# Xjh-UCAS/TAM-TR

Hardware: AMD Instinct MI355X
Metric: images/sec fwd+bwd @640x640 bs=16/GPU (higher is better)
Workload: dtype bf16

## Files before the change

### include/tamtr_hip.h

```cpp
#ifndef TAMTR_HIP_H
#define TAMTR_HIP_H

#include <stdint.h>

#ifdef __cplusplus
extern "C" {
#endif

#define TAMTR_F32 0
#define TAMTR_BF16 1

#define TAMTR_OK 0
#define TAMTR_EINVAL (-1)
#define TAMTR_EUNSUP (-2)
#define TAMTR_ELAUNCH (-3)

int tamtr_abi_version(void);

int tamtr_maxsigmoid_gate_fwd(const void* x, const float* gk, const float* bias, const void* v, void* out, float* aw,
                              int32_t* arg, int B, int nh, int hc, int HW, int T, float scale, int dtype, void* stream);

int tamtr_maxsigmoid_gate_bwd(const void* dout, const void* x, const float* gk, const void* v, const float* aw,
                              const int32_t* arg, void* dx, void* dv, float* dlogit, int B, int nh, int hc, int HW, int T,
                              float scale, int dtype, void* stream);
// ... 13 lines not shown
int tamtr_msdeform_attn_fwd(const void* value, const int32_t* shapes_host, const float* loc, const float* aw, void* out,
                            int B, int L, int M, int D, int Q, int nl, int P, int dtype, void* stream);

int tamtr_msdeform_attn_bwd(const void* gout, const void* value, const int32_t* shapes_host, const float* loc,
                            const float* aw, float* gvalue, float* gloc, float* gaw, int B, int L, int M, int D, int Q,
                            int nl, int P, int dtype, void* stream);

int tamtr_msdeform_attn_bwd_sorted(const void* gout, const void* value, const int32_t* shapes_host, const float* loc,
                                   const float* aw, void* gvalue, float* gloc, float* gaw, float* colw, int B, int L, int M,
                                   int D, int Q, int nl, int P, long long ldg, int dtype, void* stream);

int tamtr_contrastive_logits_fwd(const void* x, const float* w, const float* logit_scale, const float* bias, float* logits,
                                 float* xinv, float* winv, int B, int Q, int K, int C, int dtype, void* stream);

int tamtr_contrastive_bwd_slabs(int Q);
int tamtr_contrastive_logits_bwd(const float* g, const void* x, const float* w, const float* logit_scale, const float* xinv,
                                 const float* winv, void* dx, float* dwhat, int B, int Q, int K, int C, int dtype,
                                 void* stream);

int tamtr_linear_bf16(const void* X, const void* W, const float* bias, void* Y, int M, int N, int K, void* stream);

int tamtr_selfattn_fwd(const void* q, const void* k, const void* v, const uint32_t* mask_bits, void* o, float* lse, int B,
                       int Q, int nh, int dh, int ldq, int ldk, int ldv, int dtype, void* stream);
int tamtr_selfattn_bwd(const void* go, const void* q, const void* k, const void* v, const void* o, const float* lse,
                       const uint32_t* mask_bits, void* gq, void* gk, void* gv, float* delta_ws, int B, int Q, int nh, int dh,
                       int ldq, int ldk, int ldv, int dtype, void* stream);

int tamtr_selective_scan_chunk(void);
int tamtr_selective_scan_fwd(const float* u, const float* delta, const float* A, const float* Bm, const float* Cm,
                             const float* D, const float* dbias, float* y, float* hstate, int B, int K, int Dk, int N, int L,
                             int xmode, void* stream);
int tamtr_selective_scan_bwd_slabs(int Dk);
int tamtr_selective_scan_row_sums(void);
int tamtr_selective_scan_bwd(const float* gy, const float* u, const float* delta, const float* A, const float* Bm,
                             const float* Cm, const float* D, const float* dbias, const float* hstate, float* gu,
                             float* gdelta, float* grow, float* gB, float* gC, float* ws, int B, int K, int Dk, int N, int L,
                             int xmode, void* stream);

int tamtr_selective_scan_dtproj_fwd(const void* u, const float* dtr, const float* Wdt, const float* A, const float* Bm,
                                    const float* Cm, const float* D, const float* dbias, void* y, float* hstate, int B, int K,
                                    int Dk, int N, int R, int L, int xmode, int planes_bf16, void* stream);
int tamtr_selective_scan_dtproj_bwd(const void* gy, const void* u, const float* dtr, const float* Wdt, const float* A,
                                    const float* Bm, const float* Cm, const float* D, const float* dbias, const float* hstate,
                                    void* gu, void* gdelta_ws, float* gdtr, float* grow, float* gB, float* gC, float* ws, int B,
                                    int K, int Dk, int N, int R, int L, int xmode, int bf16_flags, void* stream);

int tamtr_lsap_assign(const float* cost, const int32_t* group_sizes_host, int bs, int nq, int G, int64_t* batch_idx,
                      int64_t* query_idx, int64_t* gt_idx, void* stream);

int tamtr_cpam_fwd(const void* x, const void* p, void* out, float* s2, int32_t* arg, int B, int C, int H, int W, int dtype,
                   void* stream);

int tamtr_cpam_bwd(const void* gout, const void* x, const void* p, const float* s2, const int32_t* arg, void* dx_direct,
                   void* du_ws, void* dp, int B, int C, int H, int W, int dtype, void* stream);

int tamtr_cpam_cl_fwd(const void* x, void* p, uint8_t* code, void* out, float* s2, int32_t* arg, int B, int C, int H, int W, int dtype, void* stream);
int tamtr_cpam_cl_bwd(const void* gout, const void* x, const void* p, const uint8_t* code, const float* s2, const int32_t* arg, void* dxd_ws,
                      void* du_ws, void* dp_ws, void* dx, int B, int C, int H, int W, int dtype, void* stream);

int tamtr_dwconv_silu_cross_fwd(const void* x, long long x_pixel_stride, const float* weight, const float* bias, void* u2, int B,
                                int D, int H, int W, int dtype, int plane_dtype, void* stream);
int tamtr_dwconv_tiles(int H, int W);
int tamtr_dwconv_silu_cross_bwd(const void* g2, const void* x, long long x_pixel_stride, const float* weight, const float* bias,
                                void* gx, long long gx_pixel_stride, float* ws, int B, int D, int H, int W, int dtype, int plane_dtype,
                                void* stream);

int tamtr_cross_merge_fwd(const void* y4, float* ymT, int B, int D, int H, int W, int plane_dtype, void* stream);
int tamtr_cross_merge_bwd(const float* gymT, void* g2, int B, int D, int H, int W, int plane_dtype, void* stream);

int tamtr_ln_gate_blocks(long long ntok);
int tamtr_ln_gate_fwd(const float* x, const void* xz, long long xz_token_stride, const float* gamma, const float* beta, void* out,
                      float* stats, long long ntok, int D, float eps, int dtype, void* stream);
int tamtr_ln_gate_bwd(const void* gout, const float* x, const void* xz, long long xz_token_stride, const float* gamma,
                      const float* beta, const float* stats, float* gx, void* gxz, float* partials, long long ntok, int D, int dtype,
                      void* stream);

int tamtr_sum_n(const void* const* src, int n, void* out, long long n_elems, int dtype, void* stream);

int tamtr_colsum_blocks(long long M);
int tamtr_colsum_bf16(const void* X, float* partial, long long M, int N, void* stream);
int tamtr_slab_sum_rows(const void* in, float* out, int R, long long C, int dtype, void* stream);
int tamtr_dw_slices(long long M, int N, int K);
int tamtr_dw_bf16(const void* dY, const void* X, float* part, int with_db, long long M, int N, int K, void* stream);
int tamtr_fold_add(const float* g4, const void* m0, const void* m1, float* out, int B, long long n, int dtype, void* stream);

int tamtr_layernorm_fwd(const void* x, const float* gamma, const float* beta, void* out, float* stats, long long ntok, int D,
                        float eps, int dtype, void* stream);
int tamtr_layernorm_bwd(const void* gout, const void* x, const float* gamma, const float* stats, void* gx, float* partials,
                        long long ntok, int D, int dtype, void* stream);

int tamtr_bn_slices(int B, int HW);
int tamtr_bn_act_fwd(const void* x, const float* gamma, const float* beta, float* running_mean, float* running_var, void* y,
                     float* mean_rstd, float* partials, int B, int C, int HW, float eps, float momentum, int act, int dtype, void* stream);
int tamtr_bn_act_bwd(const void* gy, const void* x, const float* gamma, const float* beta, const float* mean_rstd, void* gx,
                     float* ggamma, float* gbeta, float* partials, int B, int C, int HW, int act, int dtype, void* stream);

int tamtr_bncl_blocks(long long N, int C, int dtype);
int tamtr_bncl_act_fwd(const void* x, const float* gamma, const float* beta, float* running_mean, float* running_var, const void* residual,
                       void* y, float* mean_rstd, float* partials, long long N, int C, float eps, float momentum, int act, int dtype,
                       void* stream);
int tamtr_bncl_stats(const void* x, float* running_mean, float* running_var, float* mean_rstd, float* partials, long long N, int C, float eps,
                     float momentum, int dtype, void* stream);
int tamtr_bncl2_act_fwd(const void* x1, const float* gamma1, const float* beta1, float* running_mean1, float* running_var1, const void* x2,
                        const float* gamma2, const float* beta2, float* running_mean2, float* running_var2, void* y, float* mean_rstd,
                        float* partials, long long N, int C, float eps, float momentum, int act, int dtype, void* stream);
int tamtr_bncl2_act_bwd(const void* gy, long long ldgy, const void* x1, const void* x2, const float* gamma1, const float* beta1,
                        const float* gamma2, const float* beta2, const float* mean_rstd, void* gx1, void* gx2, float* ggamma1, float* gbeta1,
                        float* ggamma2, float* gbeta2, float* partials, long long N, int C, int act, int dtype, void* stream);
int tamtr_bncl_act_bwd(const void* gy, long long ldgy, const void* x, const float* gamma, const float* beta, const float* mean_rstd,
                       void* gx, float* ggamma, float* gbeta, float* partials, long long N, int C, int act, int dtype, void* stream);

int tamtr_relayout(const void* src, void* dst, int B, int C, int HW, int ld, int to_nhwc, int dtype, void* stream);
int tamtr_resample2(const void* src, void* dst, int B, int H, int W, int C, int mode, int dtype, void* stream);
int tamtr_copy_rows(const void* src, long long lds, void* dst, long long ldd, long long N, int C, int dtype, void* stream);
int tamtr_cat_rows(const void* const* src, const long long* lds, const int* C, int n, void* dst, long long ldd, long long N, int dtype,
                   void* stream);

int tamtr_maxpool_out(int n, int k, int s, int p);
int tamtr_maxpool_fwd(const void* x, void* y, uint8_t* code, int B, int C, int H, int W, int k, int s, int p, int nhwc, int dtype,
                      void* stream);
int tamtr_maxpool_bwd(const void* gy, const uint8_t* code, const void* addend, void* gx, int B, int C, int H, int W, int k, int s, int p, int nhwc, int dtype,
                      void* stream);

int tamtr_img_augment_u8(const uint8_t* src, const double* inv_affine, const uint8_t* luts, const int32_t* flags, float* out, int B,
                         int SH, int SW, int H, int W, int border, void* stream);

int tamtr_optim_chunk(void);
int tamtr_optim_step(const void* const* p, const void* const* m, const void* const* v, const void* const* e, const void* const* shadow, float* step,
                     const long long* numel,
                     const unsigned char* group, const int* chunk_tensor, const long long* chunk_off, const void* const* grads, int ntensors,
                     int nchunks, float* partial, float* normcoef, const float* lr, const float* wd, int ngroups, float beta1, float beta2, float eps,
                     float max_norm, float ema_decay, int do_ema, void* stream);

int tamtr_xproj_dw_slices(int L);
int tamtr_xproj_fwd(const void* u2, const void* wcat, float* dtr, float* Bs, float* Cs, int B, int D, int L, int R, int plane_dtype, void* stream);
int tamtr_xproj_bwd_dx(const void* gu, const float* gdtr, const float* gB, const float* gC, const void* wT, void* gu2, int B, int D, int L, int R,
                       int plane_dtype, void* stream);
int tamtr_xproj_bwd_dw(const void* u2, const float* gdtr, const float* gB, const float* gC, float* part, int B, int D, int L, int R, int plane_dtype,
                       void* stream);

int tamtr_detr_blocks(int rows_per_layer);
int tamtr_detr_layers_fwd(const float* pb, const float* ps, const float* gt_bboxes, const long long* gt_cls, const long long* li, const long long* bi,
                          const long long* si, const long long* gi, int Lr, int B, int nq, int nc, int n, long long* tgt, float* score, float* pair_l1,
                          float* pair_riou, float* partial, float g_class, float g_bbox, float g_giou, float* out, void* stream);
int tamtr_detr_layers_bwd(const float* pb, const float* ps, const float* gt_bboxes, const long long* li, const long long* bi, const long long* si,
                          const long long* gi, const long long* tgt, const float* score, const float* up, int Lr, int B, int nq, int nc, int n,
                          float g_class, float g_bbox, float g_giou, float* gpb, float* gps, void* stream);
int tamtr_detr_match_cost(const float* ps, const float* pb, const float* gt_bboxes, const long long* gt_cls, long long rows, int nc, int G, float g_class,
                          float g_bbox, float g_giou, float alpha, float gamma, float* C, void* stream);

int tamtr_bncl_act_seg_fwd(const void* x, const float* gamma, const float* beta, float* running_mean, float* running_var, void* y, long long seg_rows,
                           long long seg_pitch, float* mean_rstd, float* partials, long long N, int C, float eps, float momentum, int act, int dtype,
                           void* stream);
int tamtr_bncl_act_seg_bwd(const void* gy, long long seg_rows, long long seg_pitch, const void* x, const float* gamma, const float* beta,
                           const float* mean_rstd, void* gx, float* ggamma, float* gbeta, float* partials, long long N, int C, int act, int dtype,
                           void* stream);

int tamtr_box_refine_fwd(const float* delta, const float* ref, float* out, long long n, void* stream);
int tamtr_box_refine_bwd(const float* gout, const float* out, const float* ref, float* gdelta, float* gref, long long n, void* stream);

int tamtr_graph_capture_census(void* stream, int* counts, int n_types);

int tamtr_detect_postprocess(const void* preds, int dtype, int B, int nq, int nd, const int32_t* orig_hw, float conf, float iou,
                             int single_cls, float max_wh, const int32_t* classes, int n_classes, float* out, int32_t* keep,
                             int32_t* counts, void* stream);

// ... 80 lines not shown
```

### tam-tr_amd/_lib.py

```python
import ctypes
import os
from ctypes import c_float, c_int, c_longlong, c_void_p

_HERE = os.path.dirname(os.path.abspath(__file__))
LIB_PATH = os.environ.get('TAMTR_HIP_LIB') or os.path.join(_HERE, 'csrc', 'libtamtr_hip.so')
ABI_VERSION = 36

F32, BF16 = 0, 1
_ERR = {-1: 'TAMTR_EINVAL (bad argument)', -2: 'TAMTR_EUNSUP (shape/dtype outside what the kernels are built for)',
        -3: 'TAMTR_ELAUNCH (HIP launch error)'}


class TamtrHipError(RuntimeError):
    pass


_P, _I, _F, _LL, _D = c_void_p, c_int, c_float, c_longlong, ctypes.c_double
_SIGS = {
    'tamtr_abi_version': [],
    'tamtr_maxsigmoid_gate_fwd': [_P, _P, _P, _P, _P, _P, _P, _I, _I, _I, _I, _I, _F, _I, _P],
    'tamtr_maxsigmoid_gate_bwd': [_P, _P, _P, _P, _P, _P, _P, _P, _P, _I, _I, _I, _I, _I, _F, _I, _P],
    'tamtr_msdeform_attn_fwd': [_P, _P, _P, _P, _P, _I, _I, _I, _I, _I, _I, _I, _I, _P],
    'tamtr_msdeform_attn_bwd': [_P, _P, _P, _P, _P, _P, _P, _P, _I, _I, _I, _I, _I, _I, _I, _I, _P],
    'tamtr_msdeform_attn_bwd_sorted': [_P, _P, _P, _P, _P, _P, _P, _P, _P, _I, _I, _I, _I, _I, _I, _I, _LL, _I, _P],
    'tamtr_contrastive_logits_fwd': [_P, _P, _P, _P, _P, _P, _P, _I, _I, _I, _I, _I, _P],
    'tamtr_contrastive_logits_bwd': [_P, _P, _P, _P, _P, _P, _P, _P, _I, _I, _I, _I, _I, _P],
    'tamtr_contrastive_bwd_slabs': [_I],
    'tamtr_linear_bf16': [_P, _P, _P, _P, _I, _I, _I, _P],
    'tamtr_selfattn_fwd': [_P, _P, _P, _P, _P, _P, _I, _I, _I, _I, _I, _I, _I, _I, _P],
    'tamtr_selfattn_bwd': [_P] * 11 + [_I, _I, _I, _I, _I, _I, _I, _I, _P],
    'tamtr_selective_scan_chunk': [],
    'tamtr_selective_scan_fwd': [_P, _P, _P, _P, _P, _P, _P, _P, _P, _I, _I, _I, _I, _I, _I, _P],
    'tamtr_selective_scan_bwd_slabs': [_I],
    'tamtr_selective_scan_row_sums': [],
    'tamtr_selective_scan_bwd': [_P] * 15 + [_I, _I, _I, _I, _I, _I, _P],
    'tamtr_selective_scan_dtproj_fwd': [_P] * 10 + [_I] * 8 + [_P],
    'tamtr_selective_scan_dtproj_bwd': [_P] * 17 + [_I] * 8 + [_P],
    'tamtr_lsap_assign': [_P, _P, _I, _I, _I, _P, _P, _P, _P],
    'tamtr_img_augment_u8': [_P, _P, _P, _P, _P, _I, _I, _I, _I, _I, _I, _P],
    'tamtr_cpam_fwd': [_P, _P, _P, _P, _P, _I, _I, _I, _I, _I, _P],
    'tamtr_cpam_cl_fwd': [_P, _P, _P, _P, _P, _P, _I, _I, _I, _I, _I, _P],
    'tamtr_cpam_bwd': [_P] * 8 + [_I, _I, _I, _I, _I, _P],
    'tamtr_cpam_cl_bwd': [_P] * 10 + [_I, _I, _I, _I, _I, _P],
    'tamtr_dwconv_silu_cross_fwd': [_P, _LL, _P, _P, _P, _I, _I, _I, _I, _I, _I, _P],
    'tamtr_dwconv_tiles': [_I, _I],
    'tamtr_cross_merge_fwd': [_P, _P, _I, _I, _I, _I, _I, _P],
    'tamtr_cross_merge_bwd': [_P, _P, _I, _I, _I, _I, _I, _P],
    'tamtr_ln_gate_blocks': [_LL],
    'tamtr_bn_slices': [_I, _I],
    'tamtr_maxpool_out': [_I, _I, _I, _I],
    'tamtr_maxpool_fwd': [_P, _P, _P, _I, _I, _I, _I, _I, _I, _I, _I, _I, _P],
    'tamtr_maxpool_bwd': [_P, _P, _P, _P, _I, _I, _I, _I, _I, _I, _I, _I, _I, _P],
    'tamtr_sum_n': [_P, _I, _P, _LL, _I, _P],
    'tamtr_colsum_blocks': [_LL],
    'tamtr_colsum_bf16': [_P, _P, _LL, _I, _P],
    'tamtr_fold_add': [_P, _P, _P, _P, _I, _LL, _I, _P],
    'tamtr_slab_sum_rows': [_P, _P, _I, _LL, _I, _P],
    'tamtr_dw_slices': [_LL, _I, _I],
    'tamtr_dw_bf16': [_P, _P, _P, _I, _LL, _I, _I, _P],
    'tamtr_graph_capture_census': [_P, _P, _I],
    'tamtr_box_refine_fwd': [_P, _P, _P, _LL, _P],
    'tamtr_box_refine_bwd': [_P, _P, _P, _P, _P, _LL, _P],
    'tamtr_bncl_act_seg_fwd': [_P, _P, _P, _P, _P, _P, _LL, _LL, _P, _P, _LL, _I, _F, _F, _I, _I, _P],
    'tamtr_bncl_act_seg_bwd': [_P, _LL, _LL, _P, _P, _P, _P, _P, _P, _P, _P, _LL, _I, _I, _I, _P],
    'tamtr_detr_blocks': [_I],
    'tamtr_detr_layers_fwd': [_P] * 8 + [_I] * 5 + [_P] * 5 + [_F, _F, _F, _P, _P],
    'tamtr_detr_layers_bwd': [_P] * 10 + [_I] * 5 + [_F, _F, _F, _P, _P, _P],
    'tamtr_detr_match_cost': [_P, _P, _P, _P, _LL, _I, _I, _F, _F, _F, _F, _F, _P, _P],
    'tamtr_xproj_dw_slices': [_I],
    'tamtr_xproj_fwd': [_P, _P, _P, _P, _P, _I, _I, _I, _I, _I, _P],
    'tamtr_xproj_bwd_dx': [_P, _P, _P, _P, _P, _P, _I, _I, _I, _I, _I, _P],
    'tamtr_xproj_bwd_dw': [_P, _P, _P, _P, _P, _I, _I, _I, _I, _I, _P],
    'tamtr_optim_chunk': [],
    'tamtr_optim_step': [_P] * 11 + [_I, _I, _P, _P, _P, _P, _I, _F, _F, _F, _F, _F, _I, _P],
    'tamtr_resample2': [_P, _P, _I, _I, _I, _I, _I, _I, _P],
    'tamtr_cat_rows': [_P, _P, _P, _I, _P, _LL, _LL, _I, _P],
    'tamtr_copy_rows': [_P, _LL, _P, _LL, _LL, _I, _I, _P],
    'tamtr_relayout': [_P, _P, _I, _I, _I, _I, _I, _I, _P],
    'tamtr_bncl_blocks': [_LL, _I, _I],
    'tamtr_bncl_act_fwd': [_P, _P, _P, _P, _P, _P, _P, _P, _P, _LL, _I, _F, _F, _I, _I, _P],
    'tamtr_bncl_stats': [_P, _P, _P, _P, _P, _LL, _I, _F, _F, _I, _P],
    'tamtr_bn_finalize': [_P, _P, _P, _P, _I, _I, _F, _F, _P],
    'tamtr_conv3x3_tiles': [_I, _I, _I],
    'tamtr_conv3x3_pack_weight': [_P, _P, _I, _I, _I, _P],
    'tamtr_conv3x3_cl_stats_fwd': [_P, _LL, _P, _P, _P, _P, _P, _P, _I, _I, _I, _I, _I, _F, _F, _P],
    'tamtr_maxsigmoid_gate_cl_fwd': [_P, _LL, _P, _P, _P, _P, _P, _P, _P, _P, _P, _P, _P, _P, _I, _I, _I, _I, _I, _F, _I, _P],
    'tamtr_bncl2_act_fwd': [_P, _P, _P, _P, _P, _P, _P, _P, _P, _P, _P, _P, _P, _LL, _I, _F, _F, _I, _I, _P],
    'tamtr_bncl2_act_bwd': [_P, _LL, _P, _P, _P, _P, _P, _P, _P, _P, _P, _P, _P, _P, _P, _P, _LL, _I, _I, _I, _P],
    'tamtr_bncl_act_bwd': [_P, _LL, _P, _P, _P, _P, _P, _P, _P, _P, _LL, _I, _I, _I, _P],
    'tamtr_bn_act_fwd': [_P, _P, _P, _P, _P, _P, _P, _P, _I, _I, _I, _F, _F, _I, _I, _P],
    'tamtr_bn_act_bwd': [_P, _P, _P, _P, _P, _P, _P, _P, _P, _I, _I, _I, _I, _I, _P],
    'tamtr_layernorm_fwd': [_P, _P, _P, _P, _P, _LL, _I, _F, _I, _P],
    'tamtr_layernorm_bwd': [_P, _P, _P, _P, _P, _P, _LL, _I, _I, _P],
    'tamtr_ln_gate_fwd': [_P, _P, _LL, _P, _P, _P, _P, _LL, _I, _F, _I, _P],
    'tamtr_ln_gate_bwd': [_P, _P, _P, _LL, _P, _P, _P, _P, _P, _P, _LL, _I, _I, _P],
    'tamtr_dwconv_silu_cross_bwd': [_P, _P, _LL, _P, _P, _P, _LL, _P, _I, _I, _I, _I, _I, _I, _P],
    'tamtr_detect_postprocess': [_P, _I, _I, _I, _I, _P, _F, _F, _I, _F, _P, _I, _P, _P, _P, _P],
    'tamtr_val_postprocess_match': [_P, _I, _I, _I, _I, _F, _F, _F, _I, _F, _P, _P, _P, _I, _P, _P, _P, _P, _P],
    'tamtr_val_confusion': [_P, _P, _I, _I, _I, _P, _P, _P, _I, _P, _F, _F, _P, _P],
    'tamtr_val_ap_tile': [],
    'tamtr_val_ap_curves': [_P, _P, _P, _I, _I, _P, _I] + [_P] * 10 + [_P],
    'tamtr_text_embed': [_P, _P, _P, _P, _LL, _I, _I, _I, _P],
    'tamtr_linear_f32': [_P, _P, _P, _P, _P, _I, _I, _I, _I, _P],
    'tamtr_text_pool_project': [_P, _P, _P, _P, _P, _P, _I, _I, _I, _I, _F, _I, _P],
    'tamtr_bytetrack_update': [_P, _P, _I, _I, _P, _P, _P, _P, _P, _I, _F, _F, _F, _D, _I, _P, _P, _P, _I, _P],
    'tamtr_bytetrack_workspace_bytes': [_I, _I],
    'tamtr_botsort_update': [_P, _P, _P, _I, _I, _P, _P, _P, _P, _P, _I, _F, _F, _F, _D, _I, _P, _P, _P, _I, _P],
    'tamtr_botsort_reid_update': [_P, _P, _P, _P, _I, _I, _P, _P, _P, _P, _P, _P, _I, _I, _F, _F, _F, _D, _I, _F, _D, _P, _P, _P, _I, _P],
    'tamtr_botsort_reid_workspace_bytes': [_I, _I],
    'tamtr_reid_rows': [_P, _I, _P, _P, _I, _I, _I, _I, _P, _P],
    'tamtr_gmc_workspace_bytes': [_I, _I, _I],
    'tamtr_gmc_workspace_offset': [_I, _I, _I, _I],
    'tamtr_gmc_state_bytes': [_I, _I],
    'tamtr_gmc_estimate': [_P, _P, _P, _I, _I, _I, _P, _P, _P, _P, _P, _P, _I, _I, _P],
    'tamtr_val_coco_match': [_P, _P, _I, _I, _I, _P, _P, _P, _I, _P, _P, _I, _P, _P, _P, _P, _I, _P],
    'tamtr_val_coco_workspace_bytes': [_I, _I, _I],
    'tamtr_val_coco_accumulate': [_P, _P, _P, _I, _I, _P, _P, _I, _P, _P, _P, _P, _P],
    'tamtr_mot_update': [_P, _P, _P, _P, _I, _I, _I, _I, _D, _P, _P, _P, _P, _P, _I, _I, _P, _I, _P],
    'tamtr_mot_end_sequence': [_I, _P, _P, _P, _P, _I, _I, _I, _P, _I, _P],
    'tamtr_mot_workspace_bytes': [_I, _I, _I, _I, _I],
    'tamtr_hota_update': [_P, _P, _P, _P, _I, _I, _I, _I, _D, _D, _P, _P, _P, _I, _P],
    'tamtr_hota_end_sequence': [_P, _D, _I, _I, _I, _I, _P, _P, _P, _I, _P],
    'tamtr_hota_workspace_bytes': [_I, _I, _I],
    'tamtr_trackmap_update': [_P, _P, _P, _P, _I, _I, _I, _I, _D, _P, _P, _P, _I, _P],
    'tamtr_trackmap_end_sequence': [_P, _I, _D, _I, _P, _P, _P, _I, _P],
    'tamtr_trackmap_workspace_bytes': [_I, _I, _I, _I, _I, _I],
}
EXPORTS = tuple(_SIGS)
_lib = None


def lib():
    global _lib
    if _lib is None:
        if not os.path.exists(LIB_PATH):
            raise TamtrHipError(f'{LIB_PATH} not found: build it with `python -c "import __graft_entry__ as g; g.build()"` '
                                '(hipcc --offload-arch=gfx950). There is no CPU fallback.')
        h = ctypes.CDLL(LIB_PATH)
        for name, args in _SIGS.items():
            fn = getattr(h, name)
            fn.argtypes = args
            fn.restype = c_int
# ... 35 lines not shown
```

### tam-tr_amd/ops.py

```python
import ctypes
import math

import torch

from . import _lib
from ._lib import call, dtype_code, ptr, require_gpu, stream_ptr
import os as _os

_PROJ_CONV_LIB = _os.environ.get('TAMTR_PROJ_CONV') == 'miopen'

_I, _F = ctypes.c_int, ctypes.c_float


def _c(t):
    return t if t.is_contiguous() else t.contiguous()


def _is_cl(t):
    return t.dim() == 4 and not t.is_contiguous() and t.is_contiguous(memory_format=torch.channels_last)


def is_cl(t):
    return _is_cl(t)

# ... 397 lines not shown
        gb = (gout.view(B * Q, M, D).float() * colw.view(B * Q, M, 1)).sum(0).view(N).to(b_dt) if ctx.needs_input_grad[2] else None
        return gx, gw, gb, None, gloc.to(loc_dt), gaw.to(aw_dt), None


def value_proj_msda_ok(x, lin, n_heads, Q, P):
    K, N = lin.in_features, lin.out_features
    return (x.is_cuda and x.dtype == torch.bfloat16 and x.dim() == 3 and lin.bias is not None and N % n_heads == 0 and K % 128 == 0 and N % 128 == 0
            and msda_sorted_ok(Q, P, N // n_heads) and not _MSDA_ATOMICS and _os.environ.get('TAMTR_VALUE_BIAS') != 'colsum')


def value_proj_msda(x, lin, n_heads, shapes, loc, aw):
    return _ValueProjMSDA.apply(x, lin.weight, lin.bias, [tuple(int(v) for v in s) for s in shapes], loc, aw, int(n_heads))


class _ContrastiveLogits(torch.autograd.Function):
    @staticmethod
    def forward(ctx, x, w, logit_scale, bias):
        require_gpu(x, w, logit_scale, bias)
        B, Q, C = x.shape
        K = w.shape[1]
        x = _c(x)
        w32 = _c(w.float())
        ls, bi = _c(logit_scale.float().reshape(1)), _c(bias.float().reshape(1))
        logits = torch.empty(B, Q, K, device=x.device, dtype=torch.float32)
        xinv = torch.empty(B, Q, device=x.device, dtype=torch.float32)
        winv = torch.empty(B, K, device=x.device, dtype=torch.float32)
        call('tamtr_contrastive_logits_fwd', ptr(x), ptr(w32), ptr(ls), ptr(bi), ptr(logits), ptr(xinv), ptr(winv), B, Q, K, C,
             dtype_code(x), stream_ptr())
        ctx.save_for_backward(x, w32, ls, bi, logits, xinv, winv)
        ctx.cfg = (w.dtype, logit_scale.dtype, logit_scale.shape, bias.dtype, bias.shape)
        return logits

    @staticmethod
    def backward(ctx, g):
        x, w32, ls, bi, logits, xinv, winv = ctx.saved_tensors
        w_dt, ls_dt, ls_shape, b_dt, b_shape = ctx.cfg
        B, Q, C = x.shape
        K = w32.shape[1]
        g = _c(g.float())
        dx = torch.empty_like(x)
        if K > 16:
            _atomic_fallback(f'the contrastive head backward sums d(what) with LDS atomics for K = {K} > 16 prompts (csrc/contrastive.hip)')
        slabs = _lib.lib().tamtr_contrastive_bwd_slabs(Q)
        dwhat = torch.empty(B, slabs, K, C, device=x.device, dtype=torch.float32)
        call('tamtr_contrastive_logits_bwd', ptr(g), ptr(x), ptr(w32), ptr(ls), ptr(xinv), ptr(winv), ptr(dx), ptr(dwhat), B, Q, K,
             C, dtype_code(x), stream_ptr())
        dwhat = dwhat.sum(1) if slabs > 1 else dwhat[:, 0]
        what = w32 * winv.unsqueeze(-1)
        dw = winv.unsqueeze(-1) * (dwhat - (dwhat * what).sum(-1, keepdim=True) * what)
        dls = (g * (logits - bi)).sum().reshape(ls_shape).to(ls_dt)
        dbias = g.sum().reshape(b_shape).to(b_dt)
        return dx, dw.to(w_dt), dls, dbias


def contrastive_logits(x, w, logit_scale, bias):
    return _ContrastiveLogits.apply(x, w, logit_scale, bias)


_SPLIT_MAX = int(_os.environ.get('TAMTR_SPLITK_MAX', '64'))


def _split_count(M, min_rows=2048, max_split=None):
    max_split = _SPLIT_MAX if max_split is None else max_split
    S = 1
    while S < max_split and M % (2 * S) == 0 and M // (2 * S) >= min_rows:
        S *= 2
    return S


_BMM_F32_OUT = None

_DW_OWN = _os.environ.get('TAMTR_DW_OWN') != '0'
_DW_OWN_MAX_ROWS = 8192


def _dw_own_slices(g2, x2):
    if not (_DW_OWN and g2.is_cuda and x2.is_cuda and g2.dtype == torch.bfloat16 and x2.dtype == torch.bfloat16 and g2.dim() == 2 and x2.dim() == 2
            and g2.shape[0] == x2.shape[0] and 0 < g2.shape[0] < _DW_OWN_MAX_ROWS and g2.is_contiguous() and x2.is_contiguous()
            and g2.data_ptr() % 16 == 0 and x2.data_ptr() % 16 == 0):
        return 0
    return _lib.lib().tamtr_dw_slices(g2.shape[0], g2.shape[1], x2.shape[1])


def _dw_own(g2, x2, S, with_db):
    M, N = g2.shape
    K = x2.shape[1]
    part = torch.empty(S, N * K + N, device=g2.device, dtype=torch.float32)
    call('tamtr_dw_bf16', ptr(g2), ptr(x2), ptr(part), int(with_db), M, N, K, stream_ptr())
    tot = slab_sum(part)
    return tot[:N * K].view(N, K), tot[N * K:]


def dw_splitk(g2, x2, min_rows=2048):
    M, N = g2.shape
    K = x2.shape[1]
    S = _dw_own_slices(g2, x2)
    if S:
        return _dw_own(g2, x2, S, False)[0]
    S = _split_count(M, min_rows)
    if S == 1:
        return (g2.t() @ x2).float()
    a, b = g2.view(S, M // S, N).transpose(1, 2), x2.view(S, M // S, K)
    global _BMM_F32_OUT
    if _BMM_F32_OUT is not False and N % 8 == 0 and K % 8 == 0:
        try:
            out = torch.bmm(a, b, out_dtype=torch.float32)
            _BMM_F32_OUT = True
            return slab_sum(out)
        except (NotImplementedError, RuntimeError, TypeError):
            if _BMM_F32_OUT:
                raise
            _BMM_F32_OUT = False
    return slab_sum(torch.bmm(a, b))


def slab_sum(t):
    R = t.shape[0]
    C = t.numel() // max(R, 1)
    if not (t.is_cuda and t.dtype in (torch.float32, torch.bfloat16) and t.is_contiguous() and R > 0 and C % 4 == 0 and t.data_ptr() % 16 == 0):
        return t.float().sum(0)
    if R == 1:
        return t[0].float()
    out = torch.empty(t.shape[1:], device=t.device, dtype=torch.float32)
    call('tamtr_slab_sum_rows', ptr(t), ptr(out), R, C, dtype_code(t), stream_ptr())
    return out


def colsum(g2):
    M, N = g2.shape
    if g2.is_cuda and g2.dtype == torch.bfloat16 and M >= 4096 and N % 8 == 0 and N <= 2048 and 256 % (N // 8) == 0 and g2.is_contiguous():
        nblk = _lib.lib().tamtr_colsum_blocks(M)
        part = torch.empty(nblk, N, device=g2.device, dtype=torch.float32)
        call('tamtr_colsum_bf16', ptr(g2), ptr(part), M, N, stream_ptr())
        return slab_sum(part)
    if g2.is_cuda and g2.dtype in (torch.float32, torch.bfloat16) and N % 4 == 0:
        return slab_sum(_c(g2))
    return g2.sum(0, dtype=torch.float32)


def bf16_shadow(p):
    s = getattr(p, '_tamtr_bf16', None)
    if s is not None:
        base = getattr(p, '_tamtr_alias_of', p)
        if s._tamtr_version == base._version and s.device == p.device and s.shape == p.shape:
            return s
    return None


def bf16_of(p):
    if p.dtype == torch.bfloat16:
        return p
    s = bf16_shadow(p)
    return s if s is not None else p.to(torch.bfloat16)


KERNEL_EVENTS = {}


def _a16(t):
    return t if t is None or t.data_ptr() % 16 == 0 else t.clone()


def _linear_bf16_fwd(x2, w16, b32):
    M, K = x2.shape
    N = w16.shape[0]
    y = torch.empty(M, N, device=x2.device, dtype=torch.bfloat16)
    x2, w16, b32 = _a16(x2), _a16(w16), _a16(b32)
    rec = KERNEL_EVENTS.get('tamtr_linear_bf16')
    if rec is not None:
        e0, e1 = torch.cuda.Event(enable_timing=True), torch.cuda.Event(enable_timing=True)
        e0.record()
    call('tamtr_linear_bf16', ptr(x2), ptr(w16), ptr(b32), ptr(y), M, N, K, stream_ptr())
    if rec is not None:
        e1.record()
        rec.append((e0, e1, 2.0 * M * N * K))
    return y


def _linear_bf16_dx(g2, w16):
    N, K = w16.shape
    if K % 128 == 0 and N % 64 == 0:
        gx = torch.empty(g2.shape[0], K, device=g2.device, dtype=torch.bfloat16)
        g2, wt = _a16(g2), _a16(_c(w16.t()))
        call('tamtr_linear_bf16', ptr(g2), ptr(wt), None, ptr(gx), g2.shape[0], K, N, stream_ptr())
        return gx
    return g2 @ w16


def _bias_rows(y, idx, b32):
    if idx.numel():
        y[:, idx] = b32.to(torch.bfloat16)


def _param_grads(g2, x2, w_dt, b_dt, need_w, need_b, min_rows=2048):
    S = _dw_own_slices(g2, x2) if need_w else 0
    if S:
        with_db = b_dt is not None and need_b
        gw, gb = _dw_own(g2, x2, S, with_db)
        return gw.to(w_dt), (gb.to(b_dt) if with_db else None)
    gw = dw_splitk(g2, x2, min_rows).to(w_dt) if need_w else None
    gb = colsum(g2).to(b_dt) if (b_dt is not None and need_b) else None
    return gw, gb


def _linear_lib_bwd(needs, gy, x, w16, x_dt, w_dt, b_dt, min_rows=2048):
    N, K = w16.shape
    g2 = _c(gy.reshape(-1, N).to(x.dtype))
    x2 = _c(x.reshape(-1, K))
    gx = (g2 @ w16).view(x.shape).to(x_dt) if needs[0] else None
    return (gx,) + _param_grads(g2, x2, w_dt, b_dt, needs[1], needs[2], min_rows)


_LM_MIN_ROWS = 256


class _LinearMaster(torch.autograd.Function):

    @staticmethod
    def forward(ctx, x, weight, bias, w16=None, b16=None):
        w16 = bf16_of(weight) if w16 is None else w16
        b16 = None if bias is None else (bf16_of(bias) if b16 is None else b16)
        x16 = x if x.dtype == torch.bfloat16 else x.to(torch.bfloat16)
        ctx.save_for_backward(x16, w16)
        ctx.cfg = (x.dtype, weight.dtype, None if bias is None else bias.dtype)
        return torch.nn.functional.linear(x16, w16, b16)

    @staticmethod
    def backward(ctx, gy):
        x16, w16 = ctx.saved_tensors
        x_dt, w_dt, b_dt = ctx.cfg
        return _linear_lib_bwd(ctx.needs_input_grad, gy, x16, w16, x_dt, w_dt, b_dt, _LM_MIN_ROWS) + (None, None)


class _LinearSplitK(torch.autograd.Function):

    @staticmethod
    def forward(ctx, x, weight, bias):
        bf = x.dtype == torch.bfloat16
        w16 = bf16_of(weight) if bf else weight.to(x.dtype)
        ctx.save_for_backward(x, w16)
        ctx.cfg = (weight.dtype, None if bias is None else bias.dtype)
        return torch.nn.functional.linear(x, w16, None if bias is None else (bf16_of(bias) if bf else bias.to(x.dtype)))

    @staticmethod
    def backward(ctx, gy):
        x, w16 = ctx.saved_tensors
        w_dt, b_dt = ctx.cfg
        return _linear_lib_bwd(ctx.needs_input_grad, gy, x, w16, x.dtype, w_dt, b_dt)


class _LinearBF16(torch.autograd.Function):

    @staticmethod
    def forward(ctx, x, weight, bias, idx):
        require_gpu(x, weight, bias)
        K = x.shape[-1]
        N = weight.shape[0]
        x2 = _c(x.reshape(-1, K))
        if x2.dtype != torch.bfloat16:
            raise _lib.TamtrHipError('linear_bf16 needs bf16 activations')
        w16 = _c(bf16_of(weight))
        b32 = _c(bias.float()) if bias is not None else None
        y = _linear_bf16_fwd(x2, w16, b32).view(*x.shape[:-1], N)
        if idx is not None:
            _bias_rows(y, idx, b32)
        ctx.save_for_backward(x2, w16, idx)
        ctx.cfg = (x.shape, weight.dtype, None if bias is None else bias.dtype)
        return y

    @staticmethod
    def backward(ctx, gy):
        x2, w16, idx = ctx.saved_tensors
        xshape, w_dt, b_dt = ctx.cfg
        N, K = w16.shape
        g2 = _c(gy.reshape(-1, N).to(torch.bfloat16))
        gx = _linear_bf16_dx(g2, w16).view(xshape) if ctx.needs_input_grad[0] else None
        masked = idx is not None and idx.numel() > 0
        gw, gb = _param_grads(g2, x2, torch.float32 if masked else w_dt, b_dt, *ctx.needs_input_grad[1:3])
        if masked and gx is not None:
            gx.index_fill_(1, idx, 0)
        if masked and gw is not None:
# ... 1941 lines not shown
```

Baseline: 218.0.

## Add split-M MFMA weight-gradient kernel for tall bf16 linear layers

Adds a new HIP kernel that computes weight gradients (dY^T X) for tall matrices (M at least 16384 rows) with bf16 inputs. It splits the rows across slices, streams tiles into LDS through a multi-stage global_load_lds ring, reads them with transposed LDS reads, accumulates with MFMA, and can fuse the bias column-sum. The per-slice fp32 partials are then reduced with the existing slab_sum. A shape heuristic routes eligible GEMMs away from the hipBLAS bmm split-K path; in exchange it adds fp32 partial buffers and heuristic tuning risk.

```diff
diff --git a/include/tamtr_hip.h b/include/tamtr_hip.h
--- a/include/tamtr_hip.h
+++ b/include/tamtr_hip.h
@@ -119,6 +119,8 @@
 int tamtr_slab_sum_rows(const void* in, float* out, int R, long long C, int dtype, void* stream);
 int tamtr_dw_slices(long long M, int N, int K);
 int tamtr_dw_bf16(const void* dY, const void* X, float* part, int with_db, long long M, int N, int K, void* stream);
+int tamtr_dw_tall_slices(long long M, int N, int K);
+int tamtr_dw_tall_bf16(const void* dY, const void* X, float* part, int with_db, long long M, int N, int K, void* stream);
 int tamtr_fold_add(const float* g4, const void* m0, const void* m1, float* out, int B, long long n, int dtype, void* stream);
 
 int tamtr_layernorm_fwd(const void* x, const float* gamma, const float* beta, void* out, float* stats, long long ntok, int D,
diff --git a/tam-tr_amd/_lib.py b/tam-tr_amd/_lib.py
--- a/tam-tr_amd/_lib.py
+++ b/tam-tr_amd/_lib.py
@@ -58,6 +58,8 @@
     'tamtr_slab_sum_rows': [_P, _P, _I, _LL, _I, _P],
     'tamtr_dw_slices': [_LL, _I, _I],
     'tamtr_dw_bf16': [_P, _P, _P, _I, _LL, _I, _I, _P],
+    'tamtr_dw_tall_slices': [_LL, _I, _I],
+    'tamtr_dw_tall_bf16': [_P, _P, _P, _I, _LL, _I, _I, _P],
     'tamtr_graph_capture_census': [_P, _P, _I],
     'tamtr_box_refine_fwd': [_P, _P, _P, _LL, _P],
     'tamtr_box_refine_bwd': [_P, _P, _P, _P, _P, _LL, _P],
diff --git a/tam-tr_amd/csrc/dwtall.hip b/tam-tr_amd/csrc/dwtall.hip
--- /dev/null
+++ b/tam-tr_amd/csrc/dwtall.hip
@@ -0,0 +1,262 @@
+#include "common.h"
+
+namespace {
+
+typedef __attribute__((address_space(3))) void lds_void;
+typedef __attribute__((address_space(1))) const void gl_void;
+typedef __bf16 bf16x8 __attribute__((ext_vector_type(8)));
+
+constexpr int DT_T = 256;
+constexpr int DT_ROWS = 32;
+constexpr int DT_SMAX = 512;
+constexpr int DT_MIN_ROWS = 256;
+constexpr int DT_FILL = 512;
+
+template <int TC>
+__device__ __forceinline__ int dt_key(int r) {
+  return TC == 64 ? ((((r >> 1) & 1) << 2) | (((r >> 3) & 1) << 1)) : (((r & 3) << 2) | (((r >> 3) & 1) << 1));
+}
+
+template <int N>
+__device__ __forceinline__ void dt_vmcnt() {
+  asm volatile("s_waitcnt vmcnt(%0)" ::"n"(N) : "memory");
+}
+template <int NL, int D>
+__device__ __forceinline__ void dt_wait_landed(int rem) {
+  if constexpr (D == 0) {
+    dt_vmcnt<0>();
+  } else {
+    if (rem >= D) dt_vmcnt<D * NL>();
+    else dt_wait_landed<NL, D - 1>(rem);
+  }
+}
+
+__device__ __forceinline__ s16x4 dt_tr(uint32_t addr) {
+  s16x4 v;
+  asm volatile("ds_read_b64_tr_b16 %0, %1" : "=v"(v) : "v"(addr) : "memory");
+  return v;
+}
+__device__ __forceinline__ void dt_reads_done() { asm volatile("s_waitcnt lgkmcnt(0)" ::: "memory"); }
+__device__ __forceinline__ bf16x8 dt_frag(s16x4 a, s16x4 b) {
+  asm volatile("" : "+v"(a), "+v"(b));
+  const s16x8 f = __builtin_shufflevector(a, b, 0, 1, 2, 3, 4, 5, 6, 7);
+  return __builtin_bit_cast(bf16x8, f);
+}
+
+template <int TN, int TK, int NST>
+__global__ __launch_bounds__(DT_T, 2) void dw_tall_kernel(const bf16_t* __restrict__ dY, const bf16_t* __restrict__ X, float* __restrict__ part,
+                                                           int with_db, long long M, int N, int K, long long rps, int n_tiles, int k_tiles, int S,
+                                                           long long pitch) {
+  extern __shared__ __attribute__((aligned(16))) unsigned char smem[];
+  constexpr int Y_BYTES = DT_ROWS * TN * 2, X_BYTES = DT_ROWS * TK * 2, ST_BYTES = Y_BYTES + X_BYTES;
+  constexpr int WNW = 2, WKW = 2, NW = WNW * WKW, T = DT_T, SN = TN / WNW, SK = TK / WKW;
+  constexpr int NI = SN / 16, KI = SK / 16;
+  constexpr int LY = TN / 16 / NW, LX = TK / 16 / NW;
+  static_assert(LY * 16 * NW == TN && LX * 16 * NW == TK && NI * 16 * WNW == TN && KI * 16 * WKW == TK && T >= TN, "tile / wave grid");
+  constexpr int NL = LY + LX;
+  constexpr int AHEAD = NST - 2;
+  static_assert(NST >= 4 && (AHEAD + 1) * NL <= 63, "ring depth");
+  const int tid = threadIdx.x, lane = tid & 63, wave = __builtin_amdgcn_readfirstlane(tid >> 6);
+  const int wn = wave / WKW, wk = wave % WKW;
+  const uint32_t lds0 = (uint32_t)(uintptr_t)(lds_void*)smem;
+  const int xcd = blockIdx.x & 7, slot = blockIdx.x >> 3;
+  int sl, nt, kt;
+  if (S >= 8) {
+    const int tiles = n_tiles * k_tiles, t = slot % tiles;
+    sl = (slot / tiles) * 8 + xcd; nt = t / k_tiles; kt = t % k_tiles;
+  } else {
+    const int unit = (slot / k_tiles) * 8 + xcd;
+    sl = unit / n_tiles; nt = unit % n_tiles; kt = slot % k_tiles;
+  }
+  if (sl >= S) return;
+  const int n0 = nt * TN, k0 = kt * TK;
+  const long long m_lo = (long long)sl * rps;
+  const long long m_hi = m_lo + rps < M ? m_lo + rps : M;
+  const int nst = (int)((m_hi - m_lo + DT_ROWS - 1) / DT_ROWS);
+  const int tail = (int)(m_hi - m_lo - (long long)(nst - 1) * DT_ROWS);
+
+  const bf16_t* ysrc[LY];
+  const bf16_t* xsrc[LX];
+  int yrow[LY], xrow[LX];
+#pragma unroll
+  for (int j = 0; j < LY; ++j) {
+    const int L = (wave * LY + j) * 64 + lane, r = L / (TN / 8), c = (L % (TN / 8)) ^ dt_key<TN>(r);
+    const int col = n0 + 8 * c;
+    yrow[j] = r;
+    ysrc[j] = dY + (col < N ? col : 0);
+  }
+#pragma unroll
+  for (int j = 0; j < LX; ++j) {
+    const int L = (wave * LX + j) * 64 + lane, r = L / (TK / 8), c = (L % (TK / 8)) ^ dt_key<TK>(r);
+    const int col = k0 + 8 * c;
+    xrow[j] = r;
+    xsrc[j] = X + (col < K ? col : 0);
+  }
+  auto issue = [&](int st) {
+    unsigned char* stage = smem + (st % NST) * ST_BYTES;
+    const long long m = m_lo + (long long)st * DT_ROWS;
+#pragma unroll
+    for (int j = 0; j < LY; ++j) {
+      const long long row = m + yrow[j] < m_hi ? m + yrow[j] : m_hi - 1;
+      __builtin_amdgcn_global_load_lds((gl_void*)(ysrc[j] + (size_t)row * N), (lds_void*)(stage + (wave * LY + j) * 1024), 16, 0, 0);
+    }
+#pragma unroll
+    for (int j = 0; j < LX; ++j) {
+      const long long row = m + xrow[j] < m_hi ? m + xrow[j] : m_hi - 1;
+      __builtin_amdgcn_global_load_lds((gl_void*)(xsrc[j] + (size_t)row * K), (lds_void*)(stage + Y_BYTES + (wave * LX + j) * 1024), 16, 0, 0);
+    }
+  };
+
+  const int fg = lane >> 4, fq = (lane >> 2) & 3, fp = lane & 3;
+  const int r0 = 8 * fg + fq, r1 = r0 + 4;
+  int ya[NI][2], xa[KI][2];
+#pragma unroll
+  for (int i = 0; i < NI; ++i) {
+    const int c = (wn * SN + i * 16) / 8 + (fp >> 1);
+    ya[i][0] = (r0 * (TN / 8) + (c ^ dt_key<TN>(r0))) * 16 + 8 * (fp & 1);
+    ya[i][1] = (r1 * (TN / 8) + (c ^ dt_key<TN>(r1))) * 16 + 8 * (fp & 1);
+  }
+#pragma unroll
+  for (int j = 0; j < KI; ++j) {
+    const int c = (wk * SK + j * 16) / 8 + (fp >> 1);
+    xa[j][0] = Y_BYTES + (r0 * (TK / 8) + (c ^ dt_key<TK>(r0))) * 16 + 8 * (fp & 1);
+    xa[j][1] = Y_BYTES + (r1 * (TK / 8) + (c ^ dt_key<TK>(r1))) * 16 + 8 * (fp & 1);
+  }
+
+  const bool do_db = with_db && kt == 0 && wk == 0;
+  float colacc[NI];
+#pragma unroll
+  for (int i = 0; i < NI; ++i) colacc[i] = 0.f;
+  f32x4 acc[NI][KI];
+#pragma unroll
+  for (int i = 0; i < NI; ++i)
+#pragma unroll
+    for (int j = 0; j < KI; ++j) acc[i][j] = f32x4{0.f, 0.f, 0.f, 0.f};
+
+#pragma unroll
+  for (int p = 0; p <= AHEAD; ++p)
+    if (p < nst) issue(p);
+
+  for (int s = 0; s < nst; ++s) {
+    dt_wait_landed<NL, AHEAD>(nst - 1 - s);
+    __builtin_amdgcn_s_barrier();
+    unsigned char* st = smem + (s % NST) * ST_BYTES;
+    if (s == nst - 1 && tail < DT_ROWS) {
+      for (int o = tail * (TN * 2) + tid * 16; o < Y_BYTES; o += T * 16) *reinterpret_cast<uint4*>(st + o) = make_uint4(0, 0, 0, 0);
+      for (int o = tail * (TK * 2) + tid * 16; o < X_BYTES; o += T * 16) *reinterpret_cast<uint4*>(st + Y_BYTES + o) = make_uint4(0, 0, 0, 0);
+      __syncthreads();
+    }
+    const uint32_t sa = lds0 + (uint32_t)(s % NST) * ST_BYTES;
+    s16x4 hy[NI][2], hx[KI][2];
+#pragma unroll
+    for (int i = 0; i < NI; ++i) { hy[i][0] = dt_tr(sa + ya[i][0]); hy[i][1] = dt_tr(sa + ya[i][1]); }
+#pragma unroll
+    for (int j = 0; j < KI; ++j) { hx[j][0] = dt_tr(sa + xa[j][0]); hx[j][1] = dt_tr(sa + xa[j][1]); }
+    if (s + AHEAD + 1 < nst) issue(s + AHEAD + 1);
+    dt_reads_done();
+    bf16x8 fy[NI], fx[KI];
+#pragma unroll
+    for (int i = 0; i < NI; ++i) fy[i] = dt_frag(hy[i][0], hy[i][1]);
+#pragma unroll
+    for (int j = 0; j < KI; ++j) fx[j] = dt_frag(hx[j][0], hx[j][1]);
+    if (do_db) {
+#pragma unroll
+      for (int i = 0; i < NI; ++i)
+#pragma unroll
+        for (int e = 0; e < 8; ++e) colacc[i] += (float)fy[i][e];
+    }
+#pragma unroll
+    for (int i = 0; i < NI; ++i)
+#pragma unroll
+      for (int j = 0; j < KI; ++j) acc[i][j] = __builtin_amdgcn_mfma_f32_16x16x32_bf16(fy[i], fx[j], acc[i][j], 0, 0, 0);
+  }
+
+  float* out = part + (size_t)sl * pitch;
+  const int li = lane & 15;
+#pragma unroll
+  for (int i = 0; i < NI; ++i)
+#pragma unroll
+    for (int j = 0; j < KI; ++j) {
+      const int k = k0 + wk * SK + j * 16 + li;
+#pragma unroll
+      for (int q = 0; q < 4; ++q) {
+        const int n = n0 + wn * SN + i * 16 + 4 * fg + q;
+        if (n < N && k < K) out[(size_t)n * K + k] = acc[i][j][q];
+      }
+    }
+
+  if (kt == 0) {
+    float* red = reinterpret_cast<float*>(smem);
+    __syncthreads();
+    if (do_db) {
+#pragma unroll
+      for (int i = 0; i < NI; ++i) red[fg * TN + wn * SN + i * 16 + li] = colacc[i];
+    }
+    __syncthreads();
+    if (tid < TN && n0 + tid < N) {
+      float s = 0.f;
+      if (with_db) {
+#pragma unroll
+        for (int g = 0; g < 4; ++g) s += red[g * TN + tid];
+      }
+      out[(size_t)N * K + n0 + tid] = s;
+    }
+  }
+}
+
+struct DtPlan {
+  int tn, tk, n_tiles, k_tiles, S;
+  long long rps;
+};
+
+long long dt_rows_per_slice(long long M, long long S) { return ((M + S - 1) / S + DT_ROWS - 1) / DT_ROWS * DT_ROWS; }
+
+bool dt_plan(long long M, int N, int K, DtPlan* p) {
+  if (M <= 0 || N <= 0 || K <= 0 || N % 16 || K % 16 || N > 16384 || K > 16384 || M > (1LL << 40)) return false;
+  const int tn = N >= 128 ? 128 : 64, tk = K >= 128 ? 128 : 64;
+  const long long t = (long long)((N + tn - 1) / tn) * ((K + tk - 1) / tk);
+  long long min_rows = (4LL * N * K / (N + K) + DT_ROWS - 1) / DT_ROWS * DT_ROWS;
+  min_rows = min_rows < DT_MIN_ROWS ? DT_MIN_ROWS : min_rows;
+  long long smax = M / min_rows;
+  smax = smax < 1 ? 1 : smax > DT_SMAX ? DT_SMAX : smax;
+  long long S = (DT_FILL + t - 1) / t;
+  S = S < 1 ? 1 : S > smax ? smax : S;
+  for (;;) {
+    const long long rows = dt_rows_per_slice(M, S), s2 = (M + rows - 1) / rows;
+    if (s2 == S) break;
+    S = s2;
+  }
+  p->tn = tn; p->tk = tk;
+  p->n_tiles = (N + tn - 1) / tn; p->k_tiles = (K + tk - 1) / tk;
+  p->S = (int)S;
+  p->rps = dt_rows_per_slice(M, S);
+  return true;
+}
+
+}
+
+extern "C" int tamtr_dw_tall_slices(long long M, int N, int K) {
+  DtPlan p;
+  return dt_plan(M, N, K, &p) ? p.S : 0;
+}
+
+extern "C" int tamtr_dw_tall_bf16(const void* dY, const void* X, float* part, int with_db, long long M, int N, int K, void* stream) {
+  if (!dY || !X || !part || M <= 0 || N <= 0 || K <= 0) return TAMTR_EINVAL;
+  DtPlan p;
+  if (!dt_plan(M, N, K, &p)) return TAMTR_EUNSUP;
+  if (((uintptr_t)dY | (uintptr_t)X | (uintptr_t)part) % 16) return TAMTR_EUNSUP;
+  const long long pitch = (long long)N * K + (N + 3) / 4 * 4;
+  const long long tiles = (long long)p.n_tiles * p.k_tiles;
+  const long long groups = p.S >= 8 ? (p.S + 7) / 8 * tiles : ((long long)p.S * p.n_tiles + 7) / 8 * p.k_tiles;
+  if (groups * 8 > 0x7fffffffLL) return TAMTR_EUNSUP;
+  const dim3 grid((unsigned)(groups * 8));
+#define LAUNCH_DT(TN_, TK_, NST_)                                                                                                       \
+  hipLaunchKernelGGL((dw_tall_kernel<TN_, TK_, NST_>), grid, dim3(DT_T), (size_t)NST_ * (TN_ + TK_) * DT_ROWS * 2, (hipStream_t)stream, \
+                     (const bf16_t*)dY, (const bf16_t*)X, part, with_db, M, N, K, p.rps, p.n_tiles, p.k_tiles, p.S, pitch)
+  if (p.tn == 128 && p.tk == 128) LAUNCH_DT(128, 128, 4);
+  else if (p.tn == 128) LAUNCH_DT(128, 64, 5);
+  else if (p.tk == 128) LAUNCH_DT(64, 128, 5);
+  else LAUNCH_DT(64, 64, 6);
+#undef LAUNCH_DT
+  return tamtr_launch_status();
+}
diff --git a/tam-tr_amd/ops.py b/tam-tr_amd/ops.py
--- a/tam-tr_amd/ops.py
+++ b/tam-tr_amd/ops.py
@@ -503,11 +503,37 @@
     return _lib.lib().tamtr_dw_slices(g2.shape[0], g2.shape[1], x2.shape[1])
 
 
-def _dw_own(g2, x2, S, with_db):
+_DW_TALL = _os.environ.get('TAMTR_DW_TALL') != '0'
+_DW_TALL_MIN_ROWS = 16384
+
+
+def _dw_tall_rule(M, N, K):
+    if M < _DW_TALL_MIN_ROWS:
+        return False
+    if N < 64 and K < 64:
+        return False
+    if K > 1024 or (K >= 1024 and N >= 512):
+        return False
+    if N >= 256 and K > 256 and K & (K - 1):
+        return False
+    if min(N, K) >= 512 and M >= 65536:
+        return False
+    return True
+
+
+def _dw_tall_slices(g2, x2):
+    if not (_DW_OWN and _DW_TALL and g2.is_cuda and x2.is_cuda and g2.dtype == torch.bfloat16 and x2.dtype == torch.bfloat16 and g2.dim() == 2
+            and x2.dim() == 2 and g2.shape[0] == x2.shape[0] and g2.is_contiguous() and x2.is_contiguous()
+            and g2.data_ptr() % 16 == 0 and x2.data_ptr() % 16 == 0 and _dw_tall_rule(g2.shape[0], g2.shape[1], x2.shape[1])):
+        return 0
+    return _lib.lib().tamtr_dw_tall_slices(g2.shape[0], g2.shape[1], x2.shape[1])
+
+
+def _dw_own(g2, x2, S, with_db, entry='tamtr_dw_bf16'):
     M, N = g2.shape
     K = x2.shape[1]
     part = torch.empty(S, N * K + N, device=g2.device, dtype=torch.float32)
-    call('tamtr_dw_bf16', ptr(g2), ptr(x2), ptr(part), int(with_db), M, N, K, stream_ptr())
+    call(entry, ptr(g2), ptr(x2), ptr(part), int(with_db), M, N, K, stream_ptr())
     tot = slab_sum(part)
     return tot[:N * K].view(N, K), tot[N * K:]
 
@@ -518,6 +544,9 @@
     S = _dw_own_slices(g2, x2)
     if S:
         return _dw_own(g2, x2, S, False)[0]
+    S = _dw_tall_slices(g2, x2)
+    if S:
+        return _dw_own(g2, x2, S, False, 'tamtr_dw_tall_bf16')[0]
     S = _split_count(M, min_rows)
     if S == 1:
         return (g2.t() @ x2).float()
@@ -615,9 +644,12 @@
 
 def _param_grads(g2, x2, w_dt, b_dt, need_w, need_b, min_rows=2048):
     S = _dw_own_slices(g2, x2) if need_w else 0
+    entry = 'tamtr_dw_bf16'
+    if not S and need_w:
+        S, entry = _dw_tall_slices(g2, x2), 'tamtr_dw_tall_bf16'
     if S:
         with_db = b_dt is not None and need_b
-        gw, gb = _dw_own(g2, x2, S, with_db)
+        gw, gb = _dw_own(g2, x2, S, with_db, entry)
         return gw.to(w_dt), (gb.to(b_dt) if with_db else None)
     gw = dw_splitk(g2, x2, min_rows).to(w_dt) if need_w else None
     gb = colsum(g2).to(b_dt) if (b_dt is not None and need_b) else None
```

Result: no change. 220.0, median of 6 (+0.9%).
